# VictoriaMetrics/VictoriaMetrics

Hardware: NVIDIA H100
Metric: rollup samples/sec (block decode + rate, raw samples decoded and scanned per second) (higher is better)
Workload: dtype int64 codec -> f64 rollup

## Files before the change

victoriametrics_b200/csrc/api.cu:

```cuda
#include <cuda_runtime.h>
#include <cuda_fp16.h>
#include <stdarg.h>
#include <stdio.h>
#include <string.h>
#include <stdlib.h>

#include <algorithm>
#include <vector>

#include "common.cuh"
#include "decode.cu"
#include "rollup.cu"
#include "fused.cu"
#include "zstd.cu"
#include "marshal.inc"
#include "encode.cu"

static thread_local char g_err[512];
void vmb_set_error(const char* fmt, ...) {
    va_list ap;
    va_start(ap, fmt);
    vsnprintf(g_err, sizeof(g_err), fmt, ap);
    va_end(ap);
}
extern "C" const char* vmb_last_error(void) { return g_err; }
extern "C" int vmb_version(void) { return 100; }

#define CU(call)                                                                                   \
    do {                                                                                           \
        cudaError_t e_ = (call);                                                                   \
        if (e_ != cudaSuccess) {                                                                   \
            vmb_set_error("%s failed: %s (%s:%d)", #call, cudaGetErrorString(e_), __FILE__, __LINE__); \
            return VMB_ERR_CUDA;                                                                   \
        }                                                                                          \
    } while (0)

struct DevBuf {
    void* p = nullptr;
    size_t cap = 0;
    int reserve(size_t bytes) {
        if (bytes <= cap) return 0;
        if (p) cudaFree(p);
        p = nullptr;
        cap = 0;
        size_t want = bytes + (bytes >> 3) + 256;
        cudaError_t e = cudaMalloc(&p, want);
        if (e != cudaSuccess) {
            vmb_set_error("cudaMalloc(%zu) failed: %s", want, cudaGetErrorString(e));
            p = nullptr;
            return VMB_ERR_NOMEM;
        }
        cap = want;
        return 0;
    }
    void release() {
        if (p) cudaFree(p);
        p = nullptr;
        cap = 0;
    }
};

enum Stage { ST_ZSTD, ST_DECODE, ST_PREAMBLE, ST_ROLLUP, ST_AGGR, ST_FUSED, ST__COUNT };

#define FUSED_CHUNKS_DEFAULT 2u
#define FUSED_CHUNKS_MAX 64u

struct vmb_ctx {
    int device = 0;
    cudaStream_t stream = 0;
    uint64_t launches = 0;
    bool timing = false;
    float stage_ms[ST__COUNT] = {};
    cudaEvent_t ev[ST__COUNT] = {};
    DevBuf zseq;
    DevBuf zscratch, zlit, zstatus, zjobs, zws, args1, args2, rolled, counters, tmp_out, grp, mheap, mnext;
    DevBuf bail, sub_arrays;
    DevBuf enc_vals, enc_deltas, enc_out, enc_meta;
    DevBuf aggr_state, grp_ids;
    DevBuf oa_keys, oa_keys2, oa_cell, oa_meta;
    DevBuf cv_runs, cv_aux, cv_uniq;
    void* comm = nullptr;
    bool comm_owned = false;
    int comm_ranks = 1, comm_rank = 0;
    bool fused = true;
    uint32_t fused_chunks = 0;
    uint32_t fused_ctas_per_sm = 0;
    uint32_t huf_ctas_per_sm = 0;
    cudaStream_t zstream = nullptr;
    std::vector<cudaEvent_t> zev;
    int64_t dedup_interval = 0;
    struct vmb_series* col_cache = nullptr;
    void* h_pinned = nullptr;
    void* pipe = nullptr;
    void (*pipe_destroy)(void*) = nullptr;
};

struct vmb_blocks {
    vmb_ctx* ctx = nullptr;
    size_t nblocks = 0, nseries = 0;
    uint64_t rows = 0, compressed = 0, scratch_total = 0;
    uint64_t merge_rows = 0;
    uint64_t seq_total = 0;
    bool needs_lit = false;
    uint32_t n_huf = 0, n_gen = 0, n_bad = 0;
    uint8_t* d_arrays = nullptr;
    uint64_t* d_ser_merge_off = nullptr;
    vmb_block_desc* d_descs = nullptr;
    uint8_t* d_payload = nullptr;
    uint8_t* d_payload_alloc = nullptr;
    ColInfo* d_cols = nullptr;
    uint64_t* d_row_off = nullptr;
    uint32_t* d_huf_list = nullptr;
    uint32_t* d_gen_list = nullptr;
    uint32_t* d_bad_list = nullptr;
    uint32_t* d_ser_first = nullptr;
    uint32_t* d_ser_nblocks = nullptr;
    uint32_t* d_fused_list = nullptr;
    std::vector<uint32_t> h_fused, h_unfused, h_ser_first, h_ser_nblocks;
    std::vector<uint32_t> h_huf_upto;
    std::vector<vmb_block_desc> h_descs;
    std::vector<ColInfo> h_cols;
};

struct vmb_series {
    vmb_ctx* ctx = nullptr;
    size_t nseries = 0, nblocks = 0;
    uint64_t rows = 0;
    int64_t* d_ts = nullptr;
    double* d_vals = nullptr;
    SeriesMeta* d_meta = nullptr;
    uint32_t* d_blk_lo = nullptr;
    uint32_t* d_blk_hi = nullptr;
    int32_t* d_blk_status = nullptr;
    bool stale_dropped = false, resets_removed = false;
    uint32_t pre_applied = 0;
    bool rolled = false;
    uint32_t applied_mut = 0;
    int64_t applied_max_stale = 0;
    bool values_are_int = false;
};

static inline void count_launch(vmb_ctx* c, int n = 1) { c->launches += (uint64_t)n; }
static inline size_t al16(size_t x) { return (x + 15) & ~(size_t)15; }

extern "C" int vmb_ctx_create(int device, vmb_ctx** out) {
    if (!out) return VMB_ERR_INVALID_ARG;
    int ndev = 0;
    cudaError_t e = cudaGetDeviceCount(&ndev);
    if (e != cudaSuccess || ndev == 0) {
        vmb_set_error("no CUDA device available (%s): libvmb200 has no CPU fallback", cudaGetErrorString(e));
        return VMB_ERR_CUDA;
    }
    if (device < 0 || device >= ndev) {
        vmb_set_error("device %d out of range (%d devices)", device, ndev);
        return VMB_ERR_INVALID_ARG;
    }
    CU(cudaSetDevice(device));
    cudaDeviceProp prop;
    CU(cudaGetDeviceProperties(&prop, device));
    if (prop.major != 9 || prop.minor != 0) {
        vmb_set_error("device %d is sm_%d%d; libvmb200 is built for sm_90a (H100) only", device, prop.major, prop.minor);
        return VMB_ERR_CUDA;
    }
    vmb_ctx* c = new vmb_ctx();
    c->device = device;
    c->fused = getenv("VMB_NO_FUSED") == nullptr;
    if (const char* s = getenv("VMB_FUSED_CHUNKS")) {
        const long v = atol(s);
        c->fused_chunks = v < 1 ? 1u : (v > (long)FUSED_CHUNKS_MAX ? FUSED_CHUNKS_MAX : (uint32_t)v);
    }
    if (const char* s = getenv("VMB_FUSED_CTAS_PER_SM")) {
        const long v = atol(s);
        c->fused_ctas_per_sm = v < 1 ? 1u : (v > FU_CTAS_PER_SM ? (uint32_t)FU_CTAS_PER_SM : (uint32_t)v);
    }
    if (const char* s = getenv("VMB_HUF_CTAS_PER_SM")) {
        const long v = atol(s);
        c->huf_ctas_per_sm = v < 1 ? 1u : (v > 32 ? 32u : (uint32_t)v);
    }
    for (cudaEvent_t& e : c->ev) CU(cudaEventCreate(&e));
    CU(cudaHostAlloc(&c->h_pinned, 4096, cudaHostAllocDefault));
    *out = c;
    return VMB_OK;
}
extern "C" void vmb_series_free(vmb_series* s);
extern "C" int vmb_ctx_comm_destroy(vmb_ctx* ctx);
extern "C" void vmb_ctx_destroy(vmb_ctx* c) {
    if (!c) return;
    cudaSetDevice(c->device);
    cudaStreamSynchronize(c->stream);
    vmb_ctx_comm_destroy(c);
    if (c->col_cache) vmb_series_free(c->col_cache);
    c->col_cache = nullptr;
    DevBuf* bufs[] = {&c->zscratch, &c->zlit, &c->zstatus, &c->zjobs, &c->zws, &c->args1, &c->args2, &c->rolled,
                      &c->counters, &c->tmp_out, &c->grp, &c->mheap, &c->mnext, &c->zseq, &c->bail, &c->sub_arrays, &c->aggr_state, &c->grp_ids, &c->enc_vals, &c->enc_deltas, &c->enc_out, &c->enc_meta,
                      &c->oa_keys, &c->oa_keys2, &c->oa_cell, &c->oa_meta, &c->cv_runs, &c->cv_aux, &c->cv_uniq};
    for (DevBuf* b : bufs) b->release();
    for (cudaEvent_t e : c->ev)
        if (e) cudaEventDestroy(e);
    for (cudaEvent_t e : c->zev) cudaEventDestroy(e);
    if (c->zstream) cudaStreamDestroy(c->zstream);
    if (c->h_pinned) cudaFreeHost(c->h_pinned);
    if (c->pipe && c->pipe_destroy) c->pipe_destroy(c->pipe);
    delete c;
}
extern "C" int vmb_ctx_set_stream(vmb_ctx* c, void* stream) {
    if (!c) return VMB_ERR_INVALID_ARG;
    c->stream = (cudaStream_t)stream;
    return VMB_OK;
}
extern "C" int vmb_ctx_set_dedup_interval(vmb_ctx* c, int64_t interval_ms) {
    if (!c || interval_ms < 0) return VMB_ERR_INVALID_ARG;
    c->dedup_interval = interval_ms;
    return VMB_OK;
}
extern "C" int vmb_ctx_set_fused(vmb_ctx* c, int enable) {
    if (!c) return VMB_ERR_INVALID_ARG;
    c->fused = enable != 0;
    return VMB_OK;
}
extern "C" int vmb_ctx_synchronize(vmb_ctx* c) {
    if (!c) return VMB_ERR_INVALID_ARG;
    CU(cudaSetDevice(c->device));
    CU(cudaStreamSynchronize(c->stream));
    return VMB_OK;
}
extern "C" uint64_t vmb_ctx_launch_count(const vmb_ctx* c) { return c ? c->launches : 0; }
extern "C" float vmb_ctx_last_stage_ms(const vmb_ctx* c, int stage) {
    return (c && stage >= 0 && stage < ST__COUNT) ? c->stage_ms[stage] : 0.f;
}
extern "C" int vmb_ctx_enable_stage_timing(vmb_ctx* c, int enable) {
    if (!c) return VMB_ERR_INVALID_ARG;
    c->timing = enable != 0;
    return VMB_OK;
}
extern "C" void* vmb_host_alloc(size_t bytes) {
    void* p = nullptr;
    if (cudaHostAlloc(&p, bytes ? bytes : 1, cudaHostAllocDefault) != cudaSuccess) return nullptr;
    return p;
}
extern "C" void vmb_host_free(void* p) {
    if (p) cudaFreeHost(p);
}

static inline uint64_t be_get(const uint8_t* s, int n) {
    uint64_t v = 0;
    for (int i = 0; i < n; i++) v = (v << 8) | s[i];
    return v;
}
extern "C" int vmb_block_desc_from_header(vmb_block_desc* d, const uint8_t h[81], uint8_t tsid_out[24]) {
    if (!d || !h) return VMB_ERR_INVALID_ARG;
    memset(d, 0, sizeof(*d));
    if (tsid_out) memcpy(tsid_out, h, 24);
    auto unzz = [](uint64_t u) { return (int64_t)(u >> 1) ^ -(int64_t)(u & 1); };
    d->min_ts = unzz(be_get(h + 24, 8));
    d->max_ts = unzz(be_get(h + 32, 8));
    d->first_value = unzz(be_get(h + 40, 8));
    d->ts_off = be_get(h + 48, 8);
    d->val_off = be_get(h + 56, 8);
    d->ts_size = (uint32_t)be_get(h + 64, 4);
    d->val_size = (uint32_t)be_get(h + 68, 4);
    d->rows = (uint32_t)be_get(h + 72, 4);
    uint16_t u = (uint16_t)be_get(h + 76, 2);
    d->scale = (int16_t)((int16_t)(u >> 1) ^ (int16_t)(-(int16_t)(u & 1)));
    d->ts_mt = h[78];
    d->val_mt = h[79];
    d->precision_bits = h[80];
    if (d->rows == 0 || d->rows > 16384) return VMB_ERR_ROWS;
    if (d->ts_mt > 6 || d->val_mt > 6) return VMB_ERR_MARSHAL_TYPE;
    if (d->precision_bits < 1 || d->precision_bits > 64) return VMB_ERR_INVALID_ARG;
    if (d->ts_size > 131072 || d->val_size > 131072) return VMB_ERR_INVALID_ARG;
    return VMB_OK;
}

static inline void be_put(uint8_t* d, uint64_t v, int n) {
    for (int i = 0; i < n; i++) d[i] = (uint8_t)(v >> (8 * (n - 1 - i)));
}
extern "C" int vmb_block_header_marshal(uint8_t h[81], const vmb_block_desc* d, const uint8_t tsid[24]) {
// ... 1237 lines not shown
        FUSED_CASE(VMB_RF_STDDEV)
        FUSED_CASE(VMB_RF_STDVAR)
        FUSED_CASE(VMB_RF_CHANGES)
        FUSED_CASE(VMB_RF_DERIV)
#undef FUSED_CASE
        default: FUSED_LAUNCH((k_fused_rollup<-1>), smem0); break;
    }
#undef FUSED_LAUNCH
}

static bool fused_enabled(const vmb_ctx* ctx, const vmb_blocks* b, const vmb_rollup_cfg* cfg) {
    return ctx->fused && !b->h_fused.empty() && ctx->dedup_interval == 0 && !(cfg->flags & VMB_RC_PRE_MASK);
}

static int run_unfused_subset(vmb_ctx* ctx, const vmb_blocks* b, const std::vector<uint32_t>& sub, int32_t* d_zstatus,
                              int64_t tr_min, int64_t tr_max, const vmb_rollup_cfg* cfg, int64_t points, double* d_out,
                              const Counters& c, bool dense_rows) {
    cudaStream_t st = ctx->stream;
    std::vector<vmb_block_desc> descs;
    std::vector<uint32_t> blk_map;
    BlocksPlan pl;
    for (size_t i = 0; i < sub.size(); i++) {
        const uint32_t fb = b->h_ser_first[sub[i]], nb = b->h_ser_nblocks[sub[i]];
        for (uint32_t k = 0; k < nb; k++) {
            vmb_block_desc d = b->h_descs[fb + k];
            d.series_idx = (uint32_t)i;
            descs.push_back(d);
            pl.cols.push_back(b->h_cols[2 * (size_t)(fb + k)]);
            pl.cols.push_back(b->h_cols[2 * (size_t)(fb + k) + 1]);
            blk_map.push_back(fb + k);
        }
    }
    const size_t cn = descs.size(), cs = sub.size();
    plan_layout(pl, descs.data(), cn);
    const PlanArrays L(pl, cn, cn, cs);
    std::vector<uint8_t> hs(L.bytes);
    L.pack(hs.data(), pl, descs.data());
    memcpy(L.extra_at(hs.data(), 0), blk_map.data(), cn * 4);
    memcpy(L.extra_at(hs.data(), 1), sub.data(), cs * 4);
    int rc;
    if ((rc = ctx->sub_arrays.reserve(L.bytes + 64))) return rc;
    CU(cudaMemcpyAsync(ctx->sub_arrays.p, hs.data(), L.bytes, cudaMemcpyHostToDevice, st));
    uint8_t* da = (uint8_t*)ctx->sub_arrays.p;
    vmb_blocks bv;
    bv.ctx = ctx;
    L.bind(&bv, da, pl);
    bv.d_payload = b->d_payload;
    vmb_series view;
    if ((rc = column_cache_view(ctx, &bv, &view))) return rc;
    rc = run_decode(ctx, &bv, &view, tr_min, tr_max, 0, c.d_failed, true, d_zstatus, L.extra_at(da, 0), b->d_cols);
    if (!rc) rc = run_rollup(ctx, &view, cfg, points, d_out, c.d_scanned, dense_rows ? nullptr : L.extra_at(da, 1), false);
    cudaError_t e = cudaStreamSynchronize(st);
    if (!rc && e != cudaSuccess) {
        vmb_set_error("un-fused sub-batch: %s", cudaGetErrorString(e));
        rc = VMB_ERR_CUDA;
    }
    return rc;
}

static bool aggr_fusable(int aggr_id) {
    return aggr_id == VMB_AGGR_SUM || aggr_id == VMB_AGGR_AVG || aggr_id == VMB_AGGR_COUNT || aggr_id == VMB_AGGR_GROUP ||
           aggr_id == VMB_AGGR_SUM2 || aggr_id == VMB_AGGR_MIN || aggr_id == VMB_AGGR_MAX;
}
__global__ void k_aggr_init(int aggr, double* dv, double* dc, size_t n) {
    size_t i = (size_t)blockIdx.x * blockDim.x + threadIdx.x;
    if (i >= n) return;
    dv[i] = aggr == VMB_AGGR_MIN ? D_INF : (aggr == VMB_AGGR_MAX ? -D_INF : 0.0);
    dc[i] = 0.0;
}

static int eval_fused(vmb_ctx* ctx, const vmb_blocks* b, int64_t tr_min, int64_t tr_max, const vmb_rollup_cfg* cfg, int64_t points,
                      double* d_out, const Counters& c, const AggrTarget* af) {
    cudaStream_t st = ctx->stream;
    int rc;
    if (af) {
        if ((rc = ctx->grp_ids.reserve((b->nseries + 1) * sizeof(uint32_t)))) return rc;
        CU(cudaMemcpyAsync(ctx->grp_ids.p, af->group_ids, b->nseries * sizeof(uint32_t), cudaMemcpyHostToDevice, st));
        const size_t cells = (size_t)af->ngroups * (size_t)points;
        k_aggr_init<<<(unsigned)((cells + 255) / 256), 256, 0, st>>>(af->aggr_id, af->d_values, af->d_counts, cells);
        count_launch(ctx);
    }
    const size_t nf = b->h_fused.size();
    if ((rc = ctx->bail.reserve((nf + 2) * sizeof(uint32_t)))) return rc;
    unsigned int* d_bail_count = (unsigned int*)ctx->bail.p;
    uint32_t* d_bail_list = (uint32_t*)ctx->bail.p + 2;
    FusedParams F;
    memset(&F, 0, sizeof(F));
    if ((rc = upload_cfg_args(ctx, cfg, points, &F.cfg))) return rc;
    F.descs = b->d_descs;
    F.cols = b->d_cols;
    F.payload = b->d_payload;
    F.ser_first_block = b->d_ser_first;
    F.out = d_out;
    if (af) {
        if ((rc = ctx->tmp_out.reserve((size_t)VMB_SMS * FU_CTAS_PER_SM * (size_t)points * 8))) return rc;
        F.out = (double*)ctx->tmp_out.p;
        F.aggr_values = af->d_values;
        F.aggr_counts = af->d_counts;
        F.group_ids = (const uint32_t*)ctx->grp_ids.p;
        F.aggr_id = af->aggr_id;
    }
    F.scanned = c.d_scanned;
    F.bail_list = d_bail_list;
    F.bail_count = d_bail_count;
    F.npoints = (uint32_t)points;
    F.tr_min = tr_min;
    F.tr_max = tr_max;
    const uint32_t C = fused_chunks(ctx, b);
    auto chunk_begin = [&](uint32_t k) { return (uint32_t)(nf * k / C); };
    if (C > 1) {
        if (!ctx->zstream) CU(cudaStreamCreateWithFlags(&ctx->zstream, cudaStreamNonBlocking));
        while (ctx->zev.size() < C) {
            cudaEvent_t e;
            CU(cudaEventCreateWithFlags(&e, cudaEventDisableTiming));
            ctx->zev.push_back(e);
        }
    }
    if (ctx->timing) CU(cudaEventRecord(ctx->ev[ST_ZSTD], st));
    int32_t* d_zstatus = nullptr;
    ZstdParams Z = {};
    if ((rc = run_zstd(ctx, b, &d_zstatus, C > 1 ? b->h_huf_upto[chunk_begin(1)] : UINT32_MAX, &Z))) return rc;
    if (ctx->timing) CU(cudaEventRecord(ctx->ev[ST_DECODE], st));
    struct Join {
        cudaStream_t st;
        cudaEvent_t done = nullptr;
        ~Join() {
            if (done) cudaStreamWaitEvent(st, done, 0);
        }
    } join{st};
    if (C > 1) {
        CU(cudaEventRecord(ctx->zev[0], st));
        CU(cudaStreamWaitEvent(ctx->zstream, ctx->zev[0], 0));
        for (uint32_t k = 1; k < C; k++) {
            zstd_huf_range(ctx, b, Z, b->h_huf_upto[chunk_begin(k)], b->h_huf_upto[chunk_begin(k + 1)], ctx->zstream);
            cudaError_t e = cudaEventRecord(ctx->zev[k], ctx->zstream);
            if (e == cudaSuccess) join.done = ctx->zev[k];
            CU(e);
        }
    }
    CU(cudaMemsetAsync(d_bail_count, 0, 8, st));
    F.scratch = (const uint8_t*)ctx->zscratch.p;
    F.zstd_status = d_zstatus;
    const uint32_t ctas_per_sm = fused_ctas_per_sm(ctx, C, cfg);
    for (uint32_t k = 0; k < C; k++) {
        if (k) CU(cudaStreamWaitEvent(st, ctx->zev[k], 0));
        F.ser_list = b->d_fused_list + chunk_begin(k);
        F.nlist = chunk_begin(k + 1) - chunk_begin(k);
        launch_fused(F, ctas_per_sm, st);
        count_launch(ctx);
    }
    if (ctx->timing) CU(cudaEventRecord(ctx->ev[ST_PREAMBLE], st));
    CU(cudaGetLastError());
    unsigned int* h_bail = (unsigned int*)((char*)ctx->h_pinned + PIN_BAIL);
    CU(cudaMemcpyAsync(h_bail, d_bail_count, 4, cudaMemcpyDeviceToHost, st));
    CU(cudaStreamSynchronize(st));
    std::vector<uint32_t> sub(b->h_unfused);
    if (*h_bail) {
        const size_t n0 = sub.size();
        sub.resize(n0 + *h_bail);
        CU(cudaMemcpyAsync(sub.data() + n0, d_bail_list, (size_t)*h_bail * 4, cudaMemcpyDeviceToHost, st));
        CU(cudaStreamSynchronize(st));
        std::sort(sub.begin(), sub.end());
    }
    if (ctx->timing) {
        for (float& ms : ctx->stage_ms) ms = 0.f;
        stage_span(ctx, ST_ZSTD, ST_ZSTD, ST_DECODE);
        stage_span(ctx, ST_FUSED, ST_DECODE, ST_PREAMBLE);
    }
    if (!sub.empty()) {
        if (ctx->timing) CU(cudaEventRecord(ctx->ev[ST_ROLLUP], st));
        if (!af) {
            if ((rc = run_unfused_subset(ctx, b, sub, d_zstatus, tr_min, tr_max, cfg, points, d_out, c, false))) return rc;
        } else {
            const size_t cs = sub.size(), cells = (size_t)af->ngroups * (size_t)points;
            if ((rc = ctx->rolled.reserve((cs * (size_t)points + 2 * cells) * 8 + 64))) return rc;
            double* d_rows = (double*)ctx->rolled.p;
            if ((rc = run_unfused_subset(ctx, b, sub, d_zstatus, tr_min, tr_max, cfg, points, d_rows, c, true))) return rc;
            std::vector<uint32_t> h_csr;
            uint32_t* d_csr;
            if ((rc = upload_group_csr(ctx, h_csr, af->group_ids, sub.data(), cs, af->ngroups, 0, &d_csr))) return rc;
            aggr_fold(ctx, st, *af, d_rows, d_csr, points, d_rows + cs * (size_t)points);
            CU(cudaStreamSynchronize(st));
        }
        if (ctx->timing) {
            CU(cudaEventRecord(ctx->ev[ST_AGGR], st));
            CU(cudaStreamSynchronize(st));
            stage_span(ctx, ST_DECODE, ST_ROLLUP, ST_AGGR);
        }
    }
    return 0;
}

static int eval_device(vmb_ctx* ctx, const vmb_blocks* b, int64_t tr_min, int64_t tr_max, const vmb_rollup_cfg* cfg, int64_t points,
                       double* d_out, const AggrTarget* aggr, uint64_t* samples_scanned) {
    cudaStream_t st = ctx->stream;
    const bool fused = fused_enabled(ctx, b, cfg) && (!aggr || aggr_fusable(aggr->aggr_id));
    int rc;
    std::vector<uint32_t> h_csr;
    uint32_t* d_csr = nullptr;
    if (aggr && fused) {
        for (size_t i = 0; i < b->nseries; i++)
            if (aggr->group_ids[i] >= aggr->ngroups) return group_id_error(aggr->group_ids[i], i, aggr->ngroups);
    } else if (aggr) {
        if ((rc = upload_group_csr(ctx, h_csr, aggr->group_ids, nullptr, b->nseries, aggr->ngroups, 0, &d_csr))) return rc;
    }
    Counters c;
    if ((rc = counters_zero(ctx, st, &c))) return rc;
    if (fused) {
        if ((rc = eval_fused(ctx, b, tr_min, tr_max, cfg, points, d_out, c, aggr))) return rc;
        return counters_read(ctx, st, samples_scanned);
    }
    vmb_series view;
    if ((rc = column_cache_view(ctx, b, &view))) return rc;
    if ((rc = run_decode(ctx, b, &view, tr_min, tr_max, 0, c.d_failed))) return rc;
    double* d_rows = d_out;
    if (aggr) {
        if ((rc = ctx->rolled.reserve((size_t)b->nseries * (size_t)points * 8))) return rc;
        d_rows = (double*)ctx->rolled.p;
    }
    if ((rc = run_rollup(ctx, &view, cfg, points, d_rows, c.d_scanned))) return rc;
    if (aggr) {
        aggr_fold(ctx, st, *aggr, d_rows, d_csr, points, nullptr);
        if (ctx->timing) CU(cudaEventRecord(ctx->ev[ST_FUSED], st));
    }
    rc = counters_read(ctx, st, samples_scanned);
    if (rc && rc != VMB_ERR_BLOCK_FAILED) return rc;
    if (aggr) {
        collect_stage_times(ctx, ST_PREAMBLE, ST_FUSED);
    } else if (ctx->timing) {
        collect_stage_times(ctx, ST_ZSTD, ST_AGGR);
// ... 197 lines not shown
```

victoriametrics_b200/csrc/fused.cu:

```cuda
#pragma once
#include <type_traits>

#define FU_THREADS 128
#define FU_WARPS 4
#define FU_CTAS_PER_SM 5
#define FU_CTAS_PER_SM_OVERLAP 4
#define FU_CAP 4096
#define FU_G 2
#define FU_TILE (512 * FU_G)
#define FU_FILL (FU_WARPS * FU_TILE)
#define FU_STAGE (16 + FU_FILL + 16)
#define FU_MAX_EVENTS 32

enum {
    FU_PH_SETUP,
    FU_PH_TERM,
    FU_PH_PARSE,
    FU_PH_SCAN,
    FU_PH_EMIT,
    FU_PH_RCR,
    FU_PH_POINTS,
    FU_PH_WAIT,
    FU_PH_N,
    FU_PH_FILLS = FU_PH_N,
    FU_PH_SERIES,
    FU_PH_SLOTS
};
#ifdef VMB_FUSED_PHASES
#define FU_PH_CTAS (VMB_SMS * FU_CTAS_PER_SM)
__device__ unsigned long long fu_phase_cyc[FU_PH_CTAS][FU_PH_SLOTS];
#define FU_PH(k)                                              \
    do {                                                      \
        const long long ph_c = clock64();                     \
        if (lane == 0) S.ph[w][(k)] += (unsigned long long)(ph_c - ph_t); \
        ph_t = ph_c;                                          \
    } while (0)
#define FU_PH_COUNT(k) \
    do {               \
        if (tid == 0) S.ph[0][(k)]++; \
    } while (0)
#else
#define FU_PH(k) ((void)0)
#define FU_PH_COUNT(k) ((void)0)
#endif

#ifndef VMB_FUSED_EXP
#define VMB_FUSED_EXP 0
#endif
#define FU_EXP(b) ((VMB_FUSED_EXP & (b)) != 0)

struct FusedParams {
    const vmb_block_desc* descs;
    const ColInfo* cols;
    const uint8_t* payload;
    const uint8_t* scratch;
    const int32_t* zstd_status;
    const uint32_t* ser_list;
    const uint32_t* ser_first_block;
    vmb_rollup_cfg cfg;
    double* out;
    unsigned long long* scanned;
    uint32_t* bail_list;
    unsigned int* bail_count;
    uint32_t nlist;
    uint32_t npoints;
    int64_t tr_min, tr_max;
    double* aggr_values;
    double* aggr_counts;
    const uint32_t* group_ids;
    int aggr_id;
};

namespace {

struct FuSeries {
    const uint8_t* A;
    int64_t t_org, dts, window, max_prev, dconst, first_value;
    uint32_t shift, len, n, end_al;
    int32_t start_r, step32, win32, mpi32;
    int32_t lin_k, iq0, jq0;
    double dec_e10, dec_rcp;
    double rate_D, rate_R;
    int32_t rate_dt, rate_rows, dec_mode;
    uint32_t s;
    int16_t scale;
    uint8_t bail, is_stream, delta2, do_rcr, stale_matters, lin;
};

struct FusedSmem {
    double val[FU_CAP];
    alignas(16) uint8_t stage[2][FU_STAGE];
    unsigned long long mbar[2];
    unsigned long long w_s1[FU_WARPS], w_s2[FU_WARPS];
    uint32_t w_cnt[FU_WARPS];
    double ev_amt[FU_MAX_EVENTS], ev_cum[FU_MAX_EVENTS];
    uint32_t ev_row[FU_MAX_EVENTS];
    uint32_t nev;
    uint32_t rcr_mode;
    unsigned long long nd_v, nd_d1;
    uint32_t flags;
    uint32_t flags_emit;
    unsigned long long s_part[FU_WARPS];
    unsigned long long s_thr[FU_THREADS];
    unsigned long long s_ser[FU_THREADS];
    FuSeries ser;
#ifdef VMB_FUSED_PHASES
    unsigned long long ph[FU_WARPS][FU_PH_SLOTS];
#endif
#if FU_EXP(2)
    int32_t raw32[32][FU_THREADS];
#endif
};

__device__ __forceinline__ uint32_t smem_u32(const void* p) { return (uint32_t)__cvta_generic_to_shared(p); }

__device__ __forceinline__ void mbar_init(unsigned long long* bar, uint32_t count) {
    asm volatile("mbarrier.init.shared::cta.b64 [%0], %1;" ::"r"(smem_u32(bar)), "r"(count));
}
__device__ __forceinline__ void mbar_expect_tx(unsigned long long* bar, uint32_t bytes) {
    asm volatile("mbarrier.arrive.expect_tx.shared::cta.b64 _, [%0], %1;" ::"r"(smem_u32(bar)), "r"(bytes) : "memory");
}
__device__ __forceinline__ bool mbar_try_wait(unsigned long long* bar, uint32_t parity) {
    uint32_t ok;
    asm volatile(
        "{\n"
        ".reg .pred p;\n"
        "mbarrier.try_wait.parity.shared::cta.b64 p, [%1], %2;\n"
        "selp.u32 %0, 1, 0, p;\n"
        "}\n"
        : "=r"(ok)
        : "r"(smem_u32(bar)), "r"(parity)
        : "memory");
    return ok != 0;
}
__device__ __forceinline__ void mbar_wait(unsigned long long* bar, uint32_t parity) {
    if (mbar_try_wait(bar, parity)) return;
    const long long t0 = clock64();
    while (!mbar_try_wait(bar, parity)) {
        if (clock64() - t0 > 4000000000LL) {
            if ((threadIdx.x & 31) == 0) printf("fused: TMA copy did not land (block %u warp %u parity %u)\n", blockIdx.x, threadIdx.x >> 5, parity);
            __trap();
        }
    }
}
__device__ __forceinline__ void bulk_g2s(void* dst, const void* src, uint32_t bytes, unsigned long long* bar) {
    asm volatile("cp.async.bulk.shared::cluster.global.mbarrier::complete_tx::bytes [%0], [%1], %2, [%3];" ::"r"(smem_u32(dst)),
                 "l"(src), "r"(bytes), "r"(smem_u32(bar))
                 : "memory");
}

#define FU_MASK (FU_CAP - 1)
__device__ __forceinline__ uint32_t fu_swz(uint32_t row) {
    row &= FU_MASK;
    return row ^ ((row >> 3) & 15u);
}
__device__ __forceinline__ uint32_t fu_swz_b(uint32_t row) {
    const uint32_t o = row << 3;
    return (o ^ ((o >> 3) & 0x78u)) & (uint32_t)(FU_CAP * 8 - 1);
}
__device__ __forceinline__ double fu_ld(const double* s, uint32_t row) {
    return *reinterpret_cast<const double*>(reinterpret_cast<const char*>(s) + fu_swz_b(row));
}
__device__ __forceinline__ double& fu_ref(double* s, uint32_t row) {
    return *reinterpret_cast<double*>(reinterpret_cast<char*>(s) + fu_swz_b(row));
}
__device__ __forceinline__ double fu_lds(uint32_t val_s, uint32_t row) {
    double v;
    asm volatile("ld.shared.f64 %0, [%1];" : "=d"(v) : "r"(val_s + fu_swz_b(row)));
    return v;
}
__device__ __forceinline__ void fu_sts(uint32_t val_s, uint32_t row, double v) {
    asm volatile("st.shared.f64 [%0], %1;" ::"r"(val_s + fu_swz_b(row)), "d"(v) : "memory");
}
__device__ __forceinline__ long long fu_lds_i64(uint32_t val_s, uint32_t row) {
    long long v;
    asm volatile("ld.shared.b64 %0, [%1];" : "=l"(v) : "r"(val_s + fu_swz_b(row)));
    return v;
}
__device__ __forceinline__ void fu_sts_i64(uint32_t val_s, uint32_t row, long long v) {
    asm volatile("st.shared.b64 [%0], %1;" ::"r"(val_s + fu_swz_b(row)), "l"(v) : "memory");
}
__device__ __forceinline__ double2 fu_lds2(uint32_t val_s, uint32_t row) {
    double2 v;
    asm volatile("ld.shared.v2.f64 {%0, %1}, [%2];" : "=d"(v.x), "=d"(v.y) : "r"(val_s + (fu_swz_b(row) & ~15u)));
    return v;
}
__device__ __forceinline__ void fu_sts2(uint32_t val_s, uint32_t row, double2 v) {
    asm volatile("st.shared.v2.f64 [%0], {%1, %2};" ::"r"(val_s + (fu_swz_b(row) & ~15u)), "d"(v.x), "d"(v.y) : "memory");
}
#if FU_EXP(4)
__device__ __forceinline__ double fu_lds_o(uint32_t val_s, uint32_t row) {
    double v;
    asm("ld.shared.f64 %0, [%1];" : "=d"(v) : "r"(val_s + fu_swz_b(row)));
    return v;
}
__device__ __forceinline__ void fu_sts_o(uint32_t val_s, uint32_t row, double v) {
    asm volatile("st.shared.f64 [%0], %1;" ::"r"(val_s + fu_swz_b(row)), "d"(v));
}
__device__ __forceinline__ long long fu_lds_i64_o(uint32_t val_s, uint32_t row) {
    long long v;
    asm("ld.shared.b64 %0, [%1];" : "=l"(v) : "r"(val_s + fu_swz_b(row)));
    return v;
}
#else
#define fu_lds_o fu_lds
#define fu_sts_o fu_sts
#define fu_lds_i64_o fu_lds_i64
#endif
struct FuVals {
    const double* s;
    uint32_t r;
    __device__ __forceinline__ double operator[](int32_t i) const { return fu_ld(s, r + i); }
    __device__ __forceinline__ FuVals operator+(uint32_t k) const { return FuVals{s, r + k}; }
    __device__ __forceinline__ FuVals& operator++() { r++; return *this; }
    __device__ __forceinline__ FuVals operator++(int) { FuVals o = *this; r++; return o; }
};
// ... 102 lines not shown
            o.shift = (uint32_t)((uintptr_t)src & 15u);
            o.A = src - o.shift;
            bail = o.len < n - 1;
        } else if (mt == 3) {
            bail = d.val_size != 0;
        } else if (mt == 2) {
            uint32_t used = 0;
            bail = read_single_varint(P.payload + d.val_off, d.val_size, &o.dconst, &used) != 0 || used < d.val_size;
            bail = bail || o.dconst < 0 || (uint64_t)o.dconst > (uint64_t)0x7fffffffffffffffLL / (n - 1) ||
                   (int64_t)((uint64_t)d.first_value + (uint64_t)(n - 1) * (uint64_t)o.dconst) < d.first_value;
        } else {
            bail = true;
        }
    }
    const bool want_rcr = (rc.flags & VMB_RC_REMOVE_COUNTER_RESETS) != 0;
    o.stale_matters = (rc.flags & VMB_RC_DROP_STALE_NANS) != 0 || want_rcr || (rc.flags & VMB_RC_PRE_MASK) != 0;
    bail = bail || (rc.flags & VMB_RC_PRE_MASK) != 0;
    const int64_t max_stale = rc.lookback_delta != 0 ? rc.lookback_delta + rc.window : 0;
    o.do_rcr = want_rcr && !(max_stale > 0 && dts > max_stale);
    if (!bail && o.stale_matters && d.first_value == VMB_V_STALE_NAN) bail = true;
    o.t_org = t_org;
    o.dts = dts;
    o.window = window;
    o.max_prev = max_prev;
    o.first_value = d.first_value;
    o.n = n;
    o.end_al = (uint32_t)(((uint64_t)o.shift + o.len + 15u) & ~(uint64_t)15);
    o.scale = d.scale;
    if (!bail) {
        o.start_r = (int32_t)(rc.start - t_org);
        o.step32 = (int32_t)rc.step;
        o.win32 = (int32_t)window;
        o.mpi32 = (int32_t)max_prev;
        const int32_t dt_row = (int32_t)dts;
        if (o.step32 % dt_row == 0) {
            o.lin = 1;
            o.lin_k = o.step32 / dt_row;
            o.jq0 = fu_floor_div(o.start_r, dt_row) + 1;
            o.iq0 = fu_floor_div(o.start_r - o.win32, dt_row) + 1;
        }
    }
    {
        Dec dec;
        dec.init(d.scale);
        o.dec_e10 = dec.e10;
        o.dec_rcp = dec.rcp;
        o.dec_mode = dec.mode;
    }
    o.rate_dt = -1;
    o.rate_D = o.rate_R = 1.0;
    if (!bail && (rc.func_id == VMB_RF_RATE || rc.func_id == VMB_RF_DELTA)) {
        const int32_t dt_row = (int32_t)dts;
        const int32_t rows_w = o.lin ? o.jq0 - o.iq0 : o.win32 / dt_row;
        if (rows_w >= 1 && (int64_t)rows_w * dt_row < ((int64_t)1 << 30)) {
            o.rate_rows = rows_w;
            o.rate_dt = rows_w * dt_row;
            o.rate_D = ms_to_s((int64_t)o.rate_dt);
            o.rate_R = 1.0 / o.rate_D;
            if (((unsigned long long)__double_as_longlong(o.rate_D) & 0xfffffffffffffull) == 0xfffffffffffffull) o.rate_dt = -1;
        }
    }
    o.s = s;
    o.bail = bail;
    *out = o;
}

__device__ __forceinline__ Dec fu_dec(const FuSeries& o) {
    Dec d;
    d.e10 = o.dec_e10;
    d.rcp = o.dec_rcp;
    d.mode = o.dec_mode;
    return d;
}

__device__ __forceinline__ void fu_stage_copy(FusedSmem& S, const uint8_t* A, uint32_t end_al, uint32_t fs, uint32_t bf) {
    if (fs < end_al) {
        const uint32_t lo = fs ? fs - 16u : 0u;
        const uint32_t hi = fs + FU_FILL < end_al ? fs + FU_FILL : end_al;
        mbar_expect_tx(&S.mbar[bf], hi - lo);
        bulk_g2s(&S.stage[bf][fs ? 0 : 16], A + lo, hi - lo, &S.mbar[bf]);
    }
}

__device__ void fu_series_begin(const FusedParams& P, FusedSmem& S, uint32_t s, FuSeries* ser, uint32_t bf) {
    fu_series_setup(P, s, ser);
    if (!ser->bail && ser->is_stream) fu_stage_copy(S, ser->A, ser->end_al, 0, bf);
}

}

template <int F>
__global__ void __launch_bounds__(FU_THREADS, FU_CTAS_PER_SM) k_fused_rollup(FusedParams P) {
    extern __shared__ __align__(16) unsigned char fu_raw[];
    FusedSmem& S = *reinterpret_cast<FusedSmem*>(fu_raw);
    const FuValsRW RV{S.val};
    uint32_t val_s = smem_u32(S.val);
    asm volatile("" : "+r"(val_s));
    const vmb_rollup_cfg& rc = P.cfg;
    const uint32_t tid = threadIdx.x, lane = tid & 31u, w = tid >> 5;
    S.s_thr[tid] = 0;
    uint32_t par = 0;
    uint32_t buf = 0;
    if (tid == 0) {
        mbar_init(&S.mbar[0], 1);
        mbar_init(&S.mbar[1], 1);
        asm volatile("fence.mbarrier_init.release.cluster;" ::: "memory");
    }
#ifdef VMB_FUSED_PHASES
    for (uint32_t k = tid; k < FU_WARPS * FU_PH_SLOTS; k += FU_THREADS) (&S.ph[0][0])[k] = 0;
    long long ph_t = clock64();
#endif
    __syncthreads();

    for (uint32_t li = blockIdx.x; li < P.nlist; li += gridDim.x) {
        __syncthreads();
        if (tid == 0) {
            fu_series_begin(P, S, P.ser_list[li], &S.ser, buf);
            S.flags = 0;
            S.flags_emit = 0;
            S.nev = 0;
        }
        __syncthreads();
        const FuSeries& SE = S.ser;
        bool bail = SE.bail != 0;
        const uint32_t n = SE.n;
        const bool is_stream = SE.is_stream != 0;
        const int64_t first_value = SE.first_value;
        const int32_t dt_row = (int32_t)SE.dts;
        const uint32_t nvar = n - 1;

        auto issue_copy = [&](uint32_t fs, uint32_t bf) {
            if (tid == 0) fu_stage_copy(S, SE.A, SE.end_al, fs, bf);
        };
        uint32_t fs = 0;
        bool copy_pending = !bail && is_stream;
        uint32_t N = 0;
        uint32_t base = 0, cnt = 0, p = 0;
        uint32_t gen_rows = 0;
        double corr = 0.0, prev_raw = 0.0;
        bool stream_done = !is_stream;
        if (!bail) {
            if (tid == 0) {
                S.val[0] = fu_dec(SE).conv(first_value);
                S.nd_v = (uint64_t)first_value;
                S.nd_d1 = 0;
            }
            cnt = 1;
            gen_rows = 1;
        }
        S.s_ser[tid] = tid == 0 ? n : 0u;
        __syncthreads();
        if (!bail) prev_raw = S.val[0];
        FU_PH_COUNT(FU_PH_SERIES);
        FU_PH(FU_PH_SETUP);

#if FU_EXP(1)
        unsigned long long xacc = 0;
#endif
        uint32_t guard = 0;
        while (!bail && (p < P.npoints || !stream_done)) {
            if (++guard > 200000u) {
                bail = true;
                break;
            }
            uint32_t cnt_old = cnt;
            bool progressed = false;
            if (is_stream && !stream_done) {
                FU_PH(FU_PH_POINTS);
                FU_PH_COUNT(FU_PH_FILLS);
                if (copy_pending) {
                    mbar_wait(&S.mbar[buf], (par >> buf) & 1u);
                    par ^= 1u << buf;
                    copy_pending = false;
                }
                FU_PH(fs ? FU_PH_WAIT : FU_PH_SETUP);
                const uint8_t* st = &S.stage[buf][16];
                const uint32_t end_al = SE.end_al;
                const int64_t vlo = (int64_t)SE.shift, vhi = vlo + SE.len;
                const bool delta2 = SE.delta2 != 0, do_rcr = SE.do_rcr != 0, stale_matters = SE.stale_matters != 0;
                const uint32_t off = w * FU_TILE + lane * (16u * FU_G);
                const int64_t g0 = (int64_t)fs + off;
                uint32_t t_own[FU_G], vm[FU_G], tm[FU_G], pbm[FU_G];
#pragma unroll
                for (int g = 0; g < FU_G; g++) t_own[g] = fu_term_mask16(*reinterpret_cast<const uint4*>(st + off + 16 * g));
                const uint32_t prv_w = *reinterpret_cast<const uint32_t*>(st + off - 4);
                const int64_t gw = (int64_t)fs + w * FU_TILE;
                if (gw - 16 >= vlo && gw + FU_TILE <= vhi) {
                    uint32_t t_prev = __shfl_up_sync(VMB_FULL, t_own[FU_G - 1], 1);
                    if (lane == 0) t_prev = fu_term_mask16(*reinterpret_cast<const uint4*>(st + off - 16));
#pragma unroll
                    for (int g = 0; g < FU_G; g++) {
                        vm[g] = 0xffffu;
                        tm[g] = t_own[g];
                        pbm[g] = g ? t_own[g - 1] : t_prev;
                    }
                } else {
                    const uint32_t t_prv = fu_term_mask16(*reinterpret_cast<const uint4*>(st + off - 16));
#pragma unroll
                    for (int g = 0; g < FU_G; g++) {
                        const int64_t gg = g0 + 16 * g;
                        vm[g] = fu_valid16(gg, vlo, vhi);
                        tm[g] = t_own[g] & vm[g];
                        const uint32_t pvm = fu_valid16(gg - 16, vlo, vhi);
                        pbm[g] = (((g ? t_own[g - 1] : t_prv) & pvm) | (gg - 16 < vlo ? ~pvm : 0u)) & 0xffffu;
                    }
                }
                uint32_t cl = 0;
#pragma unroll
                for (int g = 0; g < FU_G; g++) cl += (uint32_t)__popc(tm[g]);
                uint32_t incl = cl;
#pragma unroll
                for (int o = 1; o < 32; o <<= 1) {
                    uint32_t t = __shfl_up_sync(VMB_FULL, incl, o);
                    if (lane >= (uint32_t)o) incl += t;
                }
                if (lane == 31) S.w_cnt[w] = incl;
                if (tid == 0) S.nev = 0;
                FU_PH(FU_PH_TERM);
                __syncthreads();
                FU_PH(FU_PH_WAIT);
                const bool discard = p >= P.npoints;
                if (discard) { cnt = 1; cnt_old = 1; }
                uint32_t K, tot, rb;
                {
                    const uint32_t t = lane < FU_WARPS ? S.w_cnt[lane] : 0u;
                    uint32_t ic = t;
#pragma unroll
                    for (int o = 1; o < FU_WARPS; o <<= 1) {
                        const uint32_t u = __shfl_up_sync(VMB_FULL, ic, o);
                        if (lane >= (uint32_t)o) ic += u;
                    }
                    const uint32_t fits = __ballot_sync(VMB_FULL, lane < FU_WARPS && cnt + ic <= FU_CAP) & ((1u << FU_WARPS) - 1u);
                    K = (uint32_t)__ffs((int)(~fits & ((2u << FU_WARPS) - 1u))) - 1u;
                    tot = K ? __shfl_sync(VMB_FULL, ic, (int)K - 1) : 0u;
                    const uint32_t ex = __shfl_sync(VMB_FULL, ic - t, (int)(w < FU_WARPS ? w : 0));
                    rb = w < K ? ex : 0u;
                }
                if (N + tot > nvar) bail = true;
                const uint32_t fs_next = fs + K * FU_TILE;
                const bool done_after = fs_next >= end_al;
                if (!bail && K) {
                    if (!done_after) {
                        issue_copy(fs_next, buf ^ 1u);
                        copy_pending = true;
                    }
                    FU_PH(FU_PH_TERM);
                    uint64_t s1 = 0, s2 = 0;
                    const uint32_t row0 = base + cnt + rb + incl - cl;
                    bool bad = false;
                    uint32_t carry[FU_G];
                    bool lng = false;
#pragma unroll
// ... 253 lines not shown
                                        saw_stale |= ((int64_t)vv[i] == VMB_V_STALE_NAN);
                                    }
                                }
#pragma unroll
                                for (int i = 0; i < 4; i++) fu_sts_o(val_s, row0 + k + i, f[i]);
                            }
#endif
                            for (; k < cl; k += 4) {
                                uint64_t x[4], vv[4];
#pragma unroll
                                for (int i = 0; i < 4; i++) x[i] = fu_emit_raw(k + i);
#pragma unroll
                                for (int i = 0; i < 4; i++) {
                                    const uint64_t pv = v;
                                    if (k + i < cl) {
                                        if (D2) {
                                            d1 += x[i];
                                            v += d1;
                                        } else {
                                            v += x[i];
                                        }
                                        cand |= (uint32_t)((int64_t)v < (int64_t)pv) << (k + i);
                                    }
                                    vv[i] = v;
                                }
                                double f[4];
#pragma unroll
                                for (int i = 0; i < 4; i++) f[i] = dec.conv_plain((int64_t)vv[i]);
#pragma unroll
                                for (int i = 0; i < 4; i++) {
                                    if (k + i < cl) {
                                        if (vv[i] - 0x7FFFFFFFFFFFFFFEull < 3ull) {
                                            f[i] = dec.conv((int64_t)vv[i]);
                                            saw_stale |= ((int64_t)vv[i] == VMB_V_STALE_NAN);
                                        }
                                        fu_sts_o(val_s, row0 + k + i, f[i]);
                                    }
                                }
                            }
                        };
                        if (delta2) emit_run(std::true_type{});
                        else emit_run(std::false_type{});
                        if (do_rcr && cand) {
                            do {
                                const uint32_t k = (uint32_t)__ffs((int)cand) - 1u;
                                cand &= cand - 1u;
                                const double f = fu_lds(val_s, row0 + k), pf = k ? fu_lds(val_s, row0 + k - 1u) : dec.conv((int64_t)v0);
                                const double dd = f - pf;
                                if (dd < 0) {
                                    const double amt = ((-dd * 8) < pf) ? (pf - f) : pf;
                                    const uint32_t e = atomicAdd(&S.nev, 1u);
                                    if (e < FU_MAX_EVENTS) {
                                        S.ev_row[e] = row0 + k;
                                        S.ev_amt[e] = amt;
                                    }
                                }
                            } while (cand);
                        }
                        if (saw_stale && stale_matters) S.flags_emit = 1u;
                    }
                    FU_PH(FU_PH_EMIT);
                    uint64_t nV = 0, nD1 = 0;
                    if (tid == 0) {
                        nV = S.nd_v;
                        nD1 = S.nd_d1;
                        if (delta2) {
                            nV += ts2 + (uint64_t)tc * nD1;
                            nD1 += ts1;
                        } else {
                            nV += ts1;
                        }
                    }
                    N += tc;
                    cnt += tot;
                    fs = fs_next;
                    buf ^= 1u;
                    progressed = true;
                    if (done_after) {
                        stream_done = true;
                        if (N != nvar) bail = true;
                    }
                    __syncthreads();
                    FU_PH(FU_PH_WAIT);
                    if (tid == 0) {
                        S.nd_v = nV;
                        S.nd_d1 = nD1;
                    }
                    if ((S.flags | S.flags_emit) & 1u) bail = true;
                    if (stream_done && !bail) {
                        const uint32_t last_al = (uint32_t)(vhi - 1);
                        if (SE.A[last_al] >= 0x80) bail = true;
                    }
                }
            } else if (!is_stream && gen_rows < n) {
                const uint32_t take = min(n - gen_rows, (uint32_t)FU_CAP - cnt);
                for (uint32_t k = tid; k < take; k += FU_THREADS) {
                    const uint32_t r = gen_rows + k;
                    const int64_t v = (int64_t)((uint64_t)SE.first_value + (uint64_t)r * (uint64_t)SE.dconst);
                    RV[base + cnt + k] = fu_dec(SE).conv(v);
                    if (SE.stale_matters && v == VMB_V_STALE_NAN) S.flags = 1u;
                }
                progressed = take > 0;
                gen_rows += take;
                cnt += take;
                N = gen_rows - 1;
                FU_PH(FU_PH_PARSE);
                __syncthreads();
                FU_PH(FU_PH_WAIT);
                if (S.flags & 1u) bail = true;
            }
            if (bail) break;
            const bool all_rows = is_stream ? stream_done : gen_rows == n;
            if (p >= P.npoints) continue;

            if (SE.do_rcr && cnt > cnt_old) {
                const uint32_t nev = S.nev;
                const double raw_last = RV[base + cnt - 1];
                if (nev > FU_MAX_EVENTS) {
                    bail = true;
                } else if (FU_EXP(16)) {
                } else if (nev == 0 && corr != 0.0 && isfinite(corr) && fu_ld(S.val, base + cnt_old) + corr >= fu_ld(S.val, base + cnt_old - 1)) {
                    const uint32_t a0 = base + cnt_old, a1 = base + cnt;
                    if (tid == 0 && (a0 & 1u)) fu_sts(val_s, a0, fu_lds(val_s, a0) + corr);
                    if (tid == FU_THREADS - 1 && (a1 & 1u)) fu_sts(val_s, a1 - 1u, fu_lds(val_s, a1 - 1u) + corr);
                    const uint32_t m1 = a1 >> 1;
                    for (uint32_t m = ((a0 + 1u) >> 1) + tid; m < m1; m += 4 * FU_THREADS) {
                        double2 x[4];
#pragma unroll
                        for (int i = 0; i < 4; i++) x[i] = fu_lds2(val_s, 2u * (m + i * FU_THREADS));
#pragma unroll
                        for (int i = 0; i < 4; i++)
                            if (m + i * FU_THREADS < m1) fu_sts2(val_s, 2u * (m + i * FU_THREADS), make_double2(x[i].x + corr, x[i].y + corr));
                    }
                    FU_PH(FU_PH_RCR);
                    __syncthreads();
                    FU_PH(FU_PH_WAIT);
                } else if (nev || corr != 0.0) {
                    if (tid == 0) {
                        for (uint32_t a = 1; a < nev; a++) {
                            const uint32_t rr = S.ev_row[a];
                            const double aa = S.ev_amt[a];
                            int bq = (int)a - 1;
                            while (bq >= 0 && S.ev_row[bq] > rr) {
                                S.ev_row[bq + 1] = S.ev_row[bq];
                                S.ev_amt[bq + 1] = S.ev_amt[bq];
                                bq--;
                            }
                            S.ev_row[bq + 1] = rr;
                            S.ev_amt[bq + 1] = aa;
                        }
                        double c = corr;
                        bool fin = isfinite(corr);
                        for (uint32_t a = 0; a < nev; a++) {
                            c = c + S.ev_amt[a];
                            S.ev_cum[a] = c;
                            fin = fin && isfinite(c);
                        }
                        uint32_t mode = 1;
                        if (fin) {
                            const uint32_t a0 = base + cnt_old;
                            const bool ev0 = nev && S.ev_row[0] == a0;
                            bool viol = !(RV[a0] + (ev0 ? S.ev_cum[0] : corr) >= RV[a0 - 1]);
                            for (uint32_t a = ev0 ? 1u : 0u; a < nev; a++) {
                                const uint32_t r = S.ev_row[a];
                                viol |= !(RV[r] + S.ev_cum[a] >= RV[r - 1] + (a ? S.ev_cum[a - 1] : corr));
                            }
// ... 152 lines not shown
                            np[k] = fu_lds_o(val_s, (uint32_t)is_ - 1u);
                            nl[k] = fu_lds_o(val_s, (uint32_t)(is_ + rate_rows) - 1u);
                        }
#else
#pragma unroll
                        for (int k = 0; k < 4; k++) {
                            const int32_t is_ = iq0 + (int32_t)(q + k * FU_THREADS) * lin_k;
                            vp[k] = fu_lds_o(val_s, (uint32_t)is_ - 1u);
                            vl[k] = fu_lds_o(val_s, (uint32_t)(is_ + rate_rows) - 1u);
                        }
#endif
                        uint32_t rest = 0;
#pragma unroll
                        for (int k = 0; k < 4; k++) {
                            const uint32_t qk = q + k * FU_THREADS;
                            if (qk >= p_end) break;
                            const int32_t is_ = iq0 + (int32_t)qk * lin_k;
                            const double x = vl[k] - vp[k];
                            bool ok = is_ >= 1 && is_ + rate_rows <= (int32_t)n && !isnan(vp[k]);
                            double r = x;
                            if (F == VMB_RF_RATE) {
                                const uint32_t ex = ((uint32_t)__double2hiint(x) >> 20) & 0x7ffu;
                                ok = ok && (x == 0.0 || ex - 123u < 1800u);
                                const double q0 = __dmul_rn(x, rate_R);
                                const double rem = __fma_rn(-q0, rate_D, x);
                                r = x == 0.0 ? x : __fma_rn(rem, rate_R, q0);
                            }
                            if (ok) {
                                sc32 += sc_interior;
                                put(qk, r);
                            } else {
                                rest |= 1u << k;
                            }
                        }
                        while (rest) {
                            const int k = __ffs((int)rest) - 1;
                            rest &= rest - 1u;
                            point(q + (uint32_t)k * FU_THREADS);
                        }
                    }
                } else {
#pragma unroll 2
                    for (uint32_t q = p + tid; q < p_end; q += FU_THREADS) point(q);
                }
                S.s_ser[tid] += scanned + sc32;
            }
            p = p_end;
            FU_PH(FU_PH_POINTS);
            __syncthreads();
            FU_PH(FU_PH_WAIT);
            if (p >= P.npoints) continue;
            {
                uint32_t lo = lin ? (uint32_t)min(max(iq0 + (int32_t)p * lin_k, 0), (int32_t)n)
                                  : seek_ap(start_r + (int32_t)p * step32 - win32, dt_row, inv_row, n);
                lo = lo < base ? base : (lo > base + cnt ? base + cnt : lo);
                uint32_t nb = lo > base ? lo - 1 : base;
                if (nb > base + cnt - 1) nb = base + cnt - 1;
                cnt -= nb - base;
                base = nb;
            }
        }
        if (copy_pending) {
            mbar_wait(&S.mbar[buf], (par >> buf) & 1u);
            par ^= 1u << buf;
        }
#if FU_EXP(1)
        if (!bail && tid < P.npoints)
            P.out[(size_t)(P.aggr_values ? blockIdx.x : SE.s) * P.npoints + tid] = __longlong_as_double((long long)xacc);
#endif
        if (bail) {
            if (tid == 0) {
                const unsigned int e = atomicAdd(P.bail_count, 1u);
                P.bail_list[e] = SE.s;
            }
        } else {
            S.s_thr[tid] += S.s_ser[tid];
            if (P.aggr_values) {
                __syncthreads();
                const double* row = P.out + (size_t)blockIdx.x * P.npoints;
                const size_t cell0 = (size_t)P.group_ids[SE.s] * P.npoints;
                for (uint32_t q = tid; q < P.npoints; q += FU_THREADS) fu_fold(P.aggr_id, P.aggr_values, P.aggr_counts, cell0 + q, row[q]);
            }
        }
        FU_PH(FU_PH_SETUP);
    }
#ifdef VMB_FUSED_PHASES
    if (lane == 0)
        for (int k = 0; k < FU_PH_SLOTS; k++) atomicAdd(&fu_phase_cyc[blockIdx.x][k], S.ph[w][k]);
#endif
    unsigned long long scanned = S.s_thr[tid];
    __syncthreads();
#pragma unroll
    for (int o = 16; o; o >>= 1) scanned += shfl_u64(scanned, (lane_id() ^ o));
    if (lane == 0) S.s_part[w] = scanned;
    __syncthreads();
    if (tid == 0) {
        unsigned long long tot = 0;
        for (int k = 0; k < FU_WARPS; k++) tot += S.s_part[k];
        if (tot) atomicAdd(P.scanned, tot);
    }
}

#ifdef VMB_FUSED_PHASES
extern "C" int vmb_fused_phase_cycles(unsigned long long* out, int reset) {
    if (out && cudaMemcpyFromSymbol(out, fu_phase_cyc, sizeof(fu_phase_cyc)) != cudaSuccess) return -1;
    if (reset) {
        static const unsigned long long zero[FU_PH_CTAS][FU_PH_SLOTS] = {};
        if (cudaMemcpyToSymbol(fu_phase_cyc, zero, sizeof(zero)) != cudaSuccess) return -1;
    }
    return FU_PH_SLOTS * 1000 + FU_PH_CTAS;
}
#endif
```

Before: 69.33 billion.

## Precompute fused series records in a kernel, prefetch them via bulk copy with dynamic claiming

A new pre-kernel runs series setup for every listed series in parallel and writes the records to a device array. The fused kernel then prefetches the next series record with a cp.async.bulk onto a third mbarrier while the current series is still processing, and starts the next stage copy early. Work distribution moves from a static grid stride to an atomic claim counter, and the default chunk count drops from 2 to 1, removing the split zstd stream. The cost is an extra launch, more complex parity and state tracking, and a debug trap path.

```diff
diff --git a/victoriametrics_b200/csrc/api.cu b/victoriametrics_b200/csrc/api.cu
--- a/victoriametrics_b200/csrc/api.cu
+++ b/victoriametrics_b200/csrc/api.cu
@@ -62,7 +62,7 @@
 
 enum Stage { ST_ZSTD, ST_DECODE, ST_PREAMBLE, ST_ROLLUP, ST_AGGR, ST_FUSED, ST__COUNT };
 
-#define FUSED_CHUNKS_DEFAULT 2u
+#define FUSED_CHUNKS_DEFAULT 1u
 #define FUSED_CHUNKS_MAX 64u
 
 struct vmb_ctx {
@@ -75,6 +75,7 @@
     DevBuf zseq;
     DevBuf zscratch, zlit, zstatus, zjobs, zws, args1, args2, rolled, counters, tmp_out, grp, mheap, mnext;
     DevBuf bail, sub_arrays;
+    DevBuf fused_recs;
     DevBuf enc_vals, enc_deltas, enc_out, enc_meta;
     DevBuf aggr_state, grp_ids;
     DevBuf oa_keys, oa_keys2, oa_cell, oa_meta;
@@ -192,7 +193,7 @@
     if (c->col_cache) vmb_series_free(c->col_cache);
     c->col_cache = nullptr;
     DevBuf* bufs[] = {&c->zscratch, &c->zlit, &c->zstatus, &c->zjobs, &c->zws, &c->args1, &c->args2, &c->rolled,
-                      &c->counters, &c->tmp_out, &c->grp, &c->mheap, &c->mnext, &c->zseq, &c->bail, &c->sub_arrays, &c->aggr_state, &c->grp_ids, &c->enc_vals, &c->enc_deltas, &c->enc_out, &c->enc_meta,
+                      &c->counters, &c->tmp_out, &c->grp, &c->mheap, &c->mnext, &c->zseq, &c->bail, &c->sub_arrays, &c->fused_recs, &c->aggr_state, &c->grp_ids, &c->enc_vals, &c->enc_deltas, &c->enc_out, &c->enc_meta,
                       &c->oa_keys, &c->oa_keys2, &c->oa_cell, &c->oa_meta, &c->cv_runs, &c->cv_aux, &c->cv_uniq};
     for (DevBuf* b : bufs) b->release();
     for (cudaEvent_t e : c->ev)
@@ -1596,6 +1597,7 @@
     }
     const size_t nf = b->h_fused.size();
     if ((rc = ctx->bail.reserve((nf + 2) * sizeof(uint32_t)))) return rc;
+    if ((rc = ctx->fused_recs.reserve(nf * sizeof(FuSeries)))) return rc;
     unsigned int* d_bail_count = (unsigned int*)ctx->bail.p;
     uint32_t* d_bail_list = (uint32_t*)ctx->bail.p + 2;
     FusedParams F;
@@ -1617,6 +1619,7 @@
     F.scanned = c.d_scanned;
     F.bail_list = d_bail_list;
     F.bail_count = d_bail_count;
+    F.claim = d_bail_count + 1;
     F.npoints = (uint32_t)points;
     F.tr_min = tr_min;
     F.tr_max = tr_max;
@@ -1660,6 +1663,12 @@
         if (k) CU(cudaStreamWaitEvent(st, ctx->zev[k], 0));
         F.ser_list = b->d_fused_list + chunk_begin(k);
         F.nlist = chunk_begin(k + 1) - chunk_begin(k);
+        FuSeries* recs = (FuSeries*)ctx->fused_recs.p + chunk_begin(k);
+        F.recs = recs;
+        if (F.nlist) {
+            k_fused_series_records<<<(F.nlist + 127) / 128, 128, 0, st>>>(F, recs);
+            count_launch(ctx);
+        }
         launch_fused(F, ctas_per_sm, st);
         count_launch(ctx);
     }
diff --git a/victoriametrics_b200/csrc/fused.cu b/victoriametrics_b200/csrc/fused.cu
--- a/victoriametrics_b200/csrc/fused.cu
+++ b/victoriametrics_b200/csrc/fused.cu
@@ -49,31 +49,7 @@
 #endif
 #define FU_EXP(b) ((VMB_FUSED_EXP & (b)) != 0)
 
-struct FusedParams {
-    const vmb_block_desc* descs;
-    const ColInfo* cols;
-    const uint8_t* payload;
-    const uint8_t* scratch;
-    const int32_t* zstd_status;
-    const uint32_t* ser_list;
-    const uint32_t* ser_first_block;
-    vmb_rollup_cfg cfg;
-    double* out;
-    unsigned long long* scanned;
-    uint32_t* bail_list;
-    unsigned int* bail_count;
-    uint32_t nlist;
-    uint32_t npoints;
-    int64_t tr_min, tr_max;
-    double* aggr_values;
-    double* aggr_counts;
-    const uint32_t* group_ids;
-    int aggr_id;
-};
-
-namespace {
-
-struct FuSeries {
+struct alignas(16) FuSeries {
     const uint8_t* A;
     int64_t t_org, dts, window, max_prev, dconst, first_value;
     uint32_t shift, len, n, end_al;
@@ -86,11 +62,38 @@
     int16_t scale;
     uint8_t bail, is_stream, delta2, do_rcr, stale_matters, lin;
 };
+static_assert(sizeof(FuSeries) % 16 == 0, "a record is one cp.async.bulk");
+
+struct FusedParams {
+    const vmb_block_desc* descs;
+    const ColInfo* cols;
+    const uint8_t* payload;
+    const uint8_t* scratch;
+    const int32_t* zstd_status;
+    const uint32_t* ser_list;
+    const uint32_t* ser_first_block;
+    const FuSeries* recs;
+    vmb_rollup_cfg cfg;
+    double* out;
+    unsigned long long* scanned;
+    uint32_t* bail_list;
+    unsigned int* bail_count;
+    unsigned int* claim;
+    uint32_t nlist;
+    uint32_t npoints;
+    int64_t tr_min, tr_max;
+    double* aggr_values;
+    double* aggr_counts;
+    const uint32_t* group_ids;
+    int aggr_id;
+};
+
+namespace {
 
 struct FusedSmem {
     double val[FU_CAP];
     alignas(16) uint8_t stage[2][FU_STAGE];
-    unsigned long long mbar[2];
+    unsigned long long mbar[3];
     unsigned long long w_s1[FU_WARPS], w_s2[FU_WARPS];
     uint32_t w_cnt[FU_WARPS];
     double ev_amt[FU_MAX_EVENTS], ev_cum[FU_MAX_EVENTS];
@@ -98,12 +101,17 @@
     uint32_t nev;
     uint32_t rcr_mode;
     unsigned long long nd_v, nd_d1;
+    uint32_t lnext[2];
     uint32_t flags;
     uint32_t flags_emit;
     unsigned long long s_part[FU_WARPS];
     unsigned long long s_thr[FU_THREADS];
     unsigned long long s_ser[FU_THREADS];
     FuSeries ser;
+    FuSeries ser_next;
+#if FU_EXP(32)
+    FuSeries ser0;
+#endif
 #ifdef VMB_FUSED_PHASES
     unsigned long long ph[FU_WARPS][FU_PH_SLOTS];
 #endif
@@ -132,6 +140,15 @@
         : "r"(smem_u32(bar)), "r"(parity)
         : "memory");
     return ok != 0;
+}
+__device__ __noinline__ void mbar_wait_slow(unsigned long long* bar, uint32_t parity) {
+    const long long t0 = clock64();
+    while (!mbar_try_wait(bar, parity)) {
+        if (clock64() - t0 > 4000000000LL) {
+            printf("fused: series record did not land (block %u parity %u)\n", blockIdx.x, parity);
+            __trap();
+        }
+    }
 }
 __device__ __forceinline__ void mbar_wait(unsigned long long* bar, uint32_t parity) {
     if (mbar_try_wait(bar, parity)) return;
@@ -400,11 +417,12 @@
     }
 }
 
-__device__ void fu_series_begin(const FusedParams& P, FusedSmem& S, uint32_t s, FuSeries* ser, uint32_t bf) {
-    fu_series_setup(P, s, ser);
-    if (!ser->bail && ser->is_stream) fu_stage_copy(S, ser->A, ser->end_al, 0, bf);
-}
-
+}
+
+__global__ void __launch_bounds__(128) k_fused_series_records(FusedParams P, FuSeries* recs) {
+    const uint32_t li = blockIdx.x * blockDim.x + threadIdx.x;
+    if (li == 0) *P.claim = 0;
+    if (li < P.nlist) fu_series_setup(P, P.ser_list[li], recs + li);
 }
 
 template <int F>
@@ -422,6 +440,7 @@
     if (tid == 0) {
         mbar_init(&S.mbar[0], 1);
         mbar_init(&S.mbar[1], 1);
+        mbar_init(&S.mbar[2], 1);
         asm volatile("fence.mbarrier_init.release.cluster;" ::: "memory");
     }
 #ifdef VMB_FUSED_PHASES
@@ -429,11 +448,52 @@
     long long ph_t = clock64();
 #endif
     __syncthreads();
-
-    for (uint32_t li = blockIdx.x; li < P.nlist; li += gridDim.x) {
+    auto nstate = [&]() { return (par >> 3) & 3u; };
+    auto set_nstate = [&](uint32_t v) { par = (par & ~(3u << 3)) | (v << 3); };
+    auto rec_fetch = [&](uint32_t l) {
+        if (tid == 0) {
+#if FU_EXP(32)
+            if (l != blockIdx.x) {
+                const uint32_t s = P.ser_list[l];
+                S.ser_next = S.ser0;
+                S.ser_next.s = s;
+                asm volatile("mbarrier.arrive.shared::cta.b64 _, [%0];" ::"r"(smem_u32(&S.mbar[2])) : "memory");
+            } else {
+#endif
+            asm volatile("fence.proxy.async.shared::cta;" ::: "memory");
+            mbar_expect_tx(&S.mbar[2], (uint32_t)sizeof(FuSeries));
+            bulk_g2s(&S.ser_next, P.recs + l, (uint32_t)sizeof(FuSeries), &S.mbar[2]);
+#if FU_EXP(32)
+            }
+#endif
+        }
+        set_nstate(1);
+    };
+    auto first_fill = [&](uint32_t bf) {
+        if (tid == 0) {
+            if (!mbar_try_wait(&S.mbar[2], (par >> 2) & 1u)) mbar_wait_slow(&S.mbar[2], (par >> 2) & 1u);
+            if (!S.ser_next.bail && S.ser_next.is_stream) fu_stage_copy(S, S.ser_next.A, S.ser_next.end_al, 0, bf);
+        }
+        par ^= 4u;
+        set_nstate(2);
+    };
+
+    if (tid == 0) S.lnext[0] = blockIdx.x + gridDim.x;
+    uint32_t claim = 0;
+    for (uint32_t li = blockIdx.x; li < P.nlist; li = S.lnext[((par >> 5) & 1u) ^ 1u]) {
         __syncthreads();
+        const uint32_t* const lnext = &S.lnext[(par >> 5) & 1u];
+        if (tid == 0 && *lnext < P.nlist) claim = 2 * gridDim.x + atomicAdd(P.claim, 1u);
+        if (nstate() == 0) rec_fetch(li);
+        if (nstate() == 1) first_fill(buf);
+        set_nstate(0);
         if (tid == 0) {
-            fu_series_begin(P, S, P.ser_list[li], &S.ser, buf);
+#pragma unroll
+            for (uint32_t k = 0; k < sizeof(FuSeries) / 16; k++)
+                reinterpret_cast<uint4*>(&S.ser)[k] = reinterpret_cast<const uint4*>(&S.ser_next)[k];
+#if FU_EXP(32)
+            if (li == blockIdx.x) S.ser0 = S.ser_next;
+#endif
             S.flags = 0;
             S.flags_emit = 0;
             S.nev = 0;
@@ -452,6 +512,7 @@
         };
         uint32_t fs = 0;
         bool copy_pending = !bail && is_stream;
+        if (!copy_pending && *lnext < P.nlist) rec_fetch(*lnext);
         uint32_t N = 0;
         uint32_t base = 0, cnt = 0, p = 0;
         uint32_t gen_rows = 0;
@@ -486,6 +547,7 @@
             if (is_stream && !stream_done) {
                 FU_PH(FU_PH_POINTS);
                 FU_PH_COUNT(FU_PH_FILLS);
+                if (nstate() == 0 && fs + FU_FILL >= SE.end_al && *lnext < P.nlist) rec_fetch(*lnext);
                 if (copy_pending) {
                     mbar_wait(&S.mbar[buf], (par >> buf) & 1u);
                     par ^= 1u << buf;
@@ -905,6 +967,7 @@
                     }
                     __syncthreads();
                     FU_PH(FU_PH_WAIT);
+                    if (nstate() == 1 && stream_done) first_fill(buf);
                     if (tid == 0) {
                         S.nd_v = nV;
                         S.nd_d1 = nD1;
@@ -1223,6 +1286,8 @@
                 for (uint32_t q = tid; q < P.npoints; q += FU_THREADS) fu_fold(P.aggr_id, P.aggr_values, P.aggr_counts, cell0 + q, row[q]);
             }
         }
+        if (tid == 0) S.lnext[((par >> 5) & 1u) ^ 1u] = *lnext < P.nlist ? claim : P.nlist;
+        par ^= 1u << 5;
         FU_PH(FU_PH_SETUP);
     }
 #ifdef VMB_FUSED_PHASES
```

New measurement: 74.53 billion (median of 6 runs). +7.5%, better.
